# suryatmodulus/livekit-server

Measured on AMD Instinct MI355X. Metric: forwarded RTP pkts/sec per GPU & node (bit-exact) + % HBM roofline, higher is better.
Workload: dtype u8; 1 GPU; configs[1]: 100 rooms x 10 participants per GPU, VP8 3-layer simulcast + Opus, 18000 DownTracks, 2% loss, 1% reorder, layer switching; batch=1 s of media per step, step=raw datagrams -> Buffer.calc -> forward (lkf_ingest_device + lkf_run), parallelism=room-sharded x1

## Files before the change

livekit-server_amd/csrc/engine.cpp:

```cpp
#include <hip/hip_runtime.h>

#include <algorithm>
#include <chrono>
#include <cmath>
#include <cstdio>
#include <cstdlib>
#include <cstring>
#include <atomic>
#include <map>
#include <memory>
#include <mutex>
#include <string>
#include <tuple>
#include <vector>

#include "../../include/lkfwd.h"
#include "ctl_csr.h"
#include "dev_buf.h"
#include "fwd_state.h"
#include "handles.h"
#include "hip_own.h"
#include "kernels.h"

using namespace lkf;
// ... 5128 lines not shown
    HIPCHK(hipStreamSynchronize(e->ingS), "sync ingest stream");
    HIPCHK(hipStreamSynchronize(e->decS), "sync decide stream");
    release_all(e->dRsRowEng, e->dRsSlotOff, e->dRsSlotDts, e->dRsSlotSub);
    HIPCHK(e->dRsRowEng.alloc(rowEng.size()), "alloc");
    HIPCHK(e->dRsSlotOff.alloc(off.size()), "alloc");
    HIPCHK(e->dRsSlotDts.alloc(dts.size()), "alloc");
    HIPCHK(e->dRsSlotSub.alloc(sub.size()), "alloc");
    HIPCHK(hipMemcpy(e->dRsRowEng, rowEng.data(), rowEng.size() * 4, hipMemcpyHostToDevice), "copy");
    HIPCHK(hipMemcpy(e->dRsSlotOff, off.data(), off.size() * 4, hipMemcpyHostToDevice), "copy");
    HIPCHK(hipMemcpy(e->dRsSlotDts, dts.data(), dts.size() * 4, hipMemcpyHostToDevice), "copy");
    HIPCHK(hipMemcpy(e->dRsSlotSub, sub.data(), sub.size() * 8, hipMemcpyHostToDevice), "copy");
    e->rsRooms = rooms;
    e->rsK = k;
    e->rsS = s;
    e->rsGen = e->topoGen;
  }
  hipStream_t cs = reinterpret_cast<hipStream_t>(stream);
  if (e->nRooms) {
    SpeakersLaunch a;
    a.nrooms = e->nRooms;
    a.roomPartOff = e->dRoomPartOff;
    a.partId = e->dPartId;
    a.partMicOff = e->dPartMicOff;
    a.mics = e->dMics;
    a.roomId = e->dRoomId;
    a.streams = e->dStreams;
    a.hot = e->dStreamHot;
    a.nowNs = now_ns;
    a.slots = e->dSpkSlots;
    a.counts = e->dSpkCounts;
    HIPCHK(launch_speakers(e->ingS, a), "speakers");
  }
  RoomPackLaunch p;
  p.rows = rows;
  p.k = k;
  p.s = s;
  p.rowEng = e->dRsRowEng;
  p.slots = e->dSpkSlots;
  p.counts = e->dSpkCounts;
  p.slotOff = e->dRsSlotOff;
  p.slotDts = e->dRsSlotDts;
  p.slotSub = e->dRsSlotSub;
  p.cum = e->dDTCum;
  p.spk = spk;
  p.bwe = bwe;
  HIPCHK(launch_room_pack(e->ingS, e->decS, p), "room pack");
  HIPCHK(hipEventRecord(e->rsSpk, e->ingS), "event");
  HIPCHK(hipEventRecord(e->rsDec, e->decS), "event");
  HIPCHK(hipStreamWaitEvent(cs, e->rsSpk, 0), "wait");
  HIPCHK(hipStreamWaitEvent(cs, e->rsDec, 0), "wait");
  return LKF_OK;
}

int lkf_debug_svc_stats(lkf_engine *e, uint64_t out[48], int reset) {
  if (!e || !out) return LKF_EINVAL;
  int rc = drain_streams(e);
  if (rc) return rc;
  unsigned long long v[48];
  const hipError_t r = read_svc_stats(v, reset);
  for (int i = 0; i < 48; i++) out[i] = v[i];
  return r == hipSuccess ? LKF_OK : LKF_ENODEV;
}

int lkf_debug_check(lkf_engine *e, uint64_t out[4], int reset) {
  if (!out) return LKF_EINVAL;
  if (e) {
    int rc = drain_streams(e);
    if (rc) return rc;
  } else if (hipDeviceSynchronize() != hipSuccess) {
    return LKF_EHIP;
  }
  unsigned long long v[4];
  hipError_t r = read_check(v, reset);
  for (int i = 0; i < 4; i++) out[i] = v[i];
  {
    unsigned long long w[4];
    if (read_check_rtcp(w, reset) == hipSuccess && w[0]) {
      if (!out[0]) out[1] = w[1], out[2] = w[2], out[3] = w[3];
      out[0] += w[0];
    }
  }
  std::atomic<uint64_t> &ctr = e ? e->rangeViolations : gRangeViolationsAll;
  const uint64_t rv = reset ? ctr.exchange(0) : ctr.load();
  if (rv) {
    if (!out[0]) out[1] = 0xD2, out[2] = 0, out[3] = 0;
    out[0] += rv;
    return LKF_OK;
  }
  return r == hipSuccess ? LKF_OK : LKF_ENODEV;
}

int lkf_debug_dd_cursors(lkf_engine *e, uint64_t out[7]) {
  if (!e || !out || !e->ddAlloc) return LKF_EINVAL;
  STEP(quiesce(e, false));
  for (int c = 0; c < lkf_engine::kCtx; c++) {
    uint64_t u[2] = {0, 0};
    D2H(u, e->ctx[c].dDDUsed, sizeof(u), "dd cursor copy");
    out[2 * c] = u[0];
    out[2 * c + 1] = u[1] & 0xffffffffu;
  }
  out[6] = e->ctx[0].dDDArena.cap();
  return LKF_OK;
}

int lkf_debug_dd_state(lkf_engine *e, int32_t dt, uint64_t out[16]) {
  if (!e || !out || dt < 0 || size_t(dt) >= e->dtp.size() || !e->dDDState) return LKF_EINVAL;
  STEP(quiesce(e, false));
  DDState d;
  DTHot h;
  D2H(&d, e->dDDState + dt, sizeof(d), "dd state");
  D2H(&h, e->dHot + dt, sizeof(h), "hot state");
  out[0] = (d.flags & DS_CACHE_INIT) ? 1 : 0;
  out[1] = d.cBase;
// ... 59 lines not shown
```

livekit-server_amd/csrc/forward_kernels.hip:

```cpp
#include <hip/hip_runtime.h>

#include "../../include/lkfwd.h"
#ifndef LKF_SVC_STATS
#define LKF_SVC_STATS 0
#endif
#if LKF_SVC_STATS
__device__ unsigned long long g_svc[64 * 48];
#define SVC_ADD(k, v) atomicAdd(&g_svc[(blockIdx.x & 63) * 48 + (k)], (unsigned long long)(v))
#endif
#include "dd_device.h"
#include "fwd_state.h"
#include "kernels.h"
#include "sender_device.h"

namespace lkf {

using u8 = uint8_t;
using u16 = uint16_t;
using u32 = uint32_t;
using u64 = uint64_t;
using i32 = int32_t;
using i64 = int64_t;

constexpr u64 HALF64 = 1ull << 63;
constexpr i32 INVALID = -1;


#ifndef LKF_CHECKED
#define LKF_CHECKED 0
#endif
#if LKF_CHECKED
__device__ unsigned long long g_chk[4];
__device__ __noinline__ void chk_fail(u32 site, u64 idx, u64 cap) {
  if (atomicAdd(&g_chk[0], 1ull) == 0) {
    g_chk[1] = site;
    g_chk[2] = idx;
    g_chk[3] = cap;
  }
}
#define CHK(cond, site, idx, cap)                   \
  do {                                              \
    if (!(cond)) chk_fail(site, u64(idx), u64(cap)); \
  } while (0)
#else
#define CHK(cond, site, idx, cap) \
  do {                            \
  } while (0)
#endif
enum ChkSite : u32 {
  CK_DEC_DT = 1,
  CK_DEC_TRACK,
  CK_DEC_PKT,
  CK_DEC_TUPLE,
  CK_DEC_SEQ,
  CK_DEC_LAYER,
  CK_DEC_EVENT,
  CK_EMIT_POS,
  CK_EMIT_DT,
  CK_EMIT_TUPLE,
  CK_EMIT_PKT,
  CK_EMIT_ARENA,
// ... 671 lines not shown
      L.h.ptgtT = L.h.tgtT = i32(ev.a[1]);
      break;
    case LKF_CTL_PLAYOUT_ACKED:
      setf(L, F_PLAYOUT_ACKED, ev.a[0] != 0);
      break;
    case kOpLayerOffsets: {
      const u32 l = lane_id();
      if (l < 9) L.offs[l] = l < 8 ? u32(u64(ev.a[l >> 1]) >> (32 * (l & 1))) : u32(u64(ev.pad));
      break;
    }
    default:
      break;
  }
}

__device__ bool fw_sourceSwitch(Lane &L, const PktV &p, i32 layer) {
  if (!hasf(L, F_STARTED)) {
    setf(L, F_STARTED, true);
    L.h.referenceLayerSpatial = layer;
    mg_setLastSnTs(L, p.esn, p.ets);
    if (hasf(L, F_VP8)) vp8_setLast(L, p);
    return true;
  } else if (L.h.referenceLayerSpatial == INVALID) {
    L.h.referenceLayerSpatial = layer;
  }
  const u64 extLastTS = L.h.extLastTS;
  u64 extExpectedTS = extLastTS;
  u64 extRefTS = extExpectedTS;
  if (L.hasRefTS) {
    i32 ref = L.h.referenceLayerSpatial;
    if (layer < 0 || layer >= 3 || ref < 0 || ref >= 3) return false;
    const bool svc = L.codec == LKF_CODEC_VP9 || L.codec == LKF_CODEC_AV1;
    const u32 off = svc ? 0u : L.offs[ref * 3 + layer];
    if (!svc && layer != ref && off == 0) return false;
    u32 ts = u32(p.ets) + off;
    extRefTS = (extRefTS & 0xFFFFFFFF00000000ull) + u64(ts);
    u32 e32 = u32(extExpectedTS);
    if (u32(ts - e32) < (1u << 31) && ts < e32) extRefTS += (1ull << 32);
    if (u32(e32 - ts) < (1u << 31) && e32 < ts && extRefTS >= (1ull << 32)) extRefTS -= (1ull << 32);
  }
  if (hasf(L, F_HAS_EXPECTED)) {
    if (hasf(L, F_STATS_INIT)) {
      i64 diff = (p.arr - L.h.statsFirstTime) * i64(L.clockRate) / 1000000000LL;
      extExpectedTS = L.h.statsExtStartTS + u64(diff);
    } else if (L.h.preStartTime != 0) {
      i64 since = p.arr - L.h.preStartTime;
      u64 rtpDiff = u64(since * i64(L.clockRate) / 1000000000LL);
      extExpectedTS = L.h.extFirstTS + rtpDiff;
      if (L.h.refTSOffset == 0) L.h.refTSOffset = extExpectedTS - extRefTS;
    }
  }
  extRefTS += L.h.refTSOffset;
  u64 extNextTS;
  const double cr = double(L.clockRate);
  if (L.h.lastSSRC == 0) {
    double diffSeconds = double(i64(extExpectedTS - extRefTS)) / cr;
    if (diffSeconds >= 0.0) {
      if (hasf(L, F_RESUME_BEHIND) && diffSeconds > 0.2)
        extNextTS = extExpectedTS;
      else if (diffSeconds > 2.0)
        extNextTS = extExpectedTS;
      else
        extNextTS = extRefTS;
    } else {
      extNextTS = extRefTS;
    }
    setf(L, F_RESUME_BEHIND, false);
  } else {
    double diffSeconds = double(i64(extRefTS - extLastTS)) / cr;
    if (diffSeconds < 0.0) {
      if (fabs(diffSeconds) > 0.05) return false;
      extNextTS = extLastTS + 1;
    } else {
      extNextTS = extRefTS;
    }
  }
  if (i64(extNextTS - extLastTS) <= 0) extNextTS = extLastTS + 1;
  mg_updateSnTsOffsets(L, p.esn, p.ets, 1, extNextTS - extLastTS);
  if (hasf(L, F_VP8)) vp8_updateOffsets(L, p);
  return true;
}

__device__ __forceinline__ int fw_common(Lane &L, const PktV &p, i32 layer, bool marker, int &ord, u64 &osn,
                                         u64 &ots) {
  if (L.h.lastSSRC != p.ssrc) {
    if (!fw_sourceSwitch(L, p, layer)) return LKF_DROP_SWITCH;
    L.h.lastSSRC = p.ssrc;
  }
  int r = mg_update(L, p, marker, ord, osn, ots);
  if (r == MG_PADDING) return LKF_DROP_PADDING;
  if (r == MG_DUP) return LKF_DROP_DUPLICATE;
  if (r == MG_OOO_MISS) return LKF_DROP_OOO_MISS;
  return -1;
}

template <bool DDK = false>
__device__ __forceinline__ void vls_rollback(Lane &L) {
  if (DDK && hasf(L, F_DD)) {
    L.dd->mask = L.dd->prevMask;
    if (L.dd->flags & DS_HAS_PREV_MASK)
      L.dd->flags |= DS_HAS_MASK;
    else
      L.dd->flags &= ~u32(DS_HAS_MASK);
  }
  L.h.curS = L.h.prevS;
  L.h.curT = L.h.prevT;
  L.h.tgtS = L.h.ptgtS;
// ... 1015 lines not shown
__device__ __forceinline__ void pin_loaded(const uint4 &a, const uint4 &b, const uint4 &c, const uint4 &d) {
  asm volatile("" ::"v"(a.x), "v"(a.y), "v"(a.z), "v"(a.w), "v"(b.x), "v"(b.y), "v"(b.z), "v"(b.w), "v"(c.x),
               "v"(c.y), "v"(c.z), "v"(c.w), "v"(d.x), "v"(d.y), "v"(d.z), "v"(d.w));
}

__device__ __forceinline__ void relaunder(uint4 &a, uint4 &b, uint4 &c, uint4 &d) {
  asm volatile("" : "+v"(a.x), "+v"(a.y), "+v"(a.z), "+v"(a.w), "+v"(b.x), "+v"(b.y), "+v"(b.z), "+v"(b.w),
                 "+v"(c.x), "+v"(c.y), "+v"(c.z), "+v"(c.w), "+v"(d.x), "+v"(d.y), "+v"(d.z), "+v"(d.w));
}

__device__ __forceinline__ bool steady_state(const Lane &L) {
  const u32 fl = L.h.flags;
  return (fl & F_VIDEO) && (fl & F_SIMULCAST) && !(fl & (F_MUTED | F_PUBMUTED)) &&
         L.h.tgtS != INVALID && L.h.tgtT != INVALID && L.h.curS == L.h.tgtS && L.h.curS <= L.h.maxS &&
         L.h.curS >= 0 && L.h.curS < 3;
}

__global__ void __launch_bounds__(64) k_layer_index(const RunDesc *__restrict__ desc, const u32 *__restrict__ tBegin,
                                                    const u32 *__restrict__ tEnd, u32 stride, u32 *__restrict__ list,
                                                    u32 *__restrict__ before, u32 *__restrict__ cnt,
                                                    u64 *__restrict__ zero2) {
  const lkf_pkt *__restrict__ pkts = reinterpret_cast<const lkf_pkt *>(desc->pkts);
  const u32 t = blockIdx.x, lane = threadIdx.x;
  if (zero2 && t == 0 && lane < 2) zero2[lane] = 0;
  const u64 lt = (1ull << lane) - 1;
  const u32 b = tBegin[t], e = tEnd[t];
  u32 c0 = 0, c1 = 0, c2 = 0;
  for (u32 base = b; base < e; base += 64) {
    const u32 i = base + lane;
    const int l = i < e ? int(reinterpret_cast<const int8_t *>(pkts + i)[53]) : -1;
    const u64 m0 = __ballot(l == 0), m1 = __ballot(l == 1), m2 = __ballot(l == 2);
    if (i < e) {
      const u32 r0 = c0 + u32(__popcll(m0 & lt)), r1 = c1 + u32(__popcll(m1 & lt)), r2 = c2 + u32(__popcll(m2 & lt));
      before[i] = r0;
      before[stride + i] = r1;
      before[2 * size_t(stride) + i] = r2;
      if (l == 0) list[b + r0] = i;
      if (l == 1) list[stride + b + r1] = i;
      if (l == 2) list[2 * size_t(stride) + b + r2] = i;
    }
    c0 += u32(__popcll(m0));
    c1 += u32(__popcll(m1));
    c2 += u32(__popcll(m2));
  }
  if (lane == 0) {
    cnt[t * 3] = c0;
    cnt[t * 3 + 1] = c1;
    cnt[t * 3 + 2] = c2;
  }
}

#ifndef LKF_SVC_CHAINS
#define LKF_SVC_CHAINS 1
#endif
constexpr int kSvcDDBytes = 48;
constexpr int kSvcFrames = 72;
enum : u32 { SK_BAD = 0, SK_FWD = 1, SK_MDROP = 2, SK_NDROP = 3 };

#if LKF_SVC_STATS
#define SVC_WHY(c) \
  if (why == 0 && inWin && !good) why = (c)
#else
#define SVC_WHY(c)
#endif

template <bool DDK>
__device__ __forceinline__ u32 svc_run(Lane &L, LaneOut &o, const PktV &p, u32 pi, u32 n, u32 pos, u32 nextAt,
                                       bool valid, i32 &sentAcc, u8 *sScr, u8 *sFD) {
  const u32 lane = lane_id();
  const u64 lt = (1ull << lane) - 1;
  const u32 fl = L.h.flags;
  const bool inWin = valid && lane >= pos && pi < nextAt;
  const u64 winM = __ballot(inWin);
  const bool dd = DDK && (fl & F_DD);
  {
    const int ns = (fl & (F_MUTED | F_PUBMUTED)) ? LKF_DROP_MUTED
                   : (L.h.tgtS == INVALID || L.h.tgtT == INVALID) ? LKF_DROP_PAUSED
                                                                  : -1;
    if (ns >= 0) {
      const u32 k = u32(__popcll(winM));
      o.nTuples += k;
      if (ns == LKF_DROP_MUTED)
        o.drops[LKF_DROP_MUTED] += k;
      else
        o.drops[LKF_DROP_PAUSED] += k;
      return pos + k;
    }
  }
  const bool curValid = L.h.curS != INVALID && L.h.curT != INVALID;
  const bool started = fl & F_STARTED;
  const bool relevantDrop = curValid && started;
  bool uni = true;
  const DDStruct *s = nullptr;
  int hiPos = -1, maxTgt = -1;
  u32 hiTarget = 0;
  bool swAll = false;
  u32 aboveM = 0, hiChain = 0xffffffffu;
  if (DDK && dd) {
    const DDState &d = *L.dd;
    uni = (d.flags & DS_KF_VALID) && (d.flags & DS_CACHE_INIT);
    uni = uni && u32(d.slot) == L.ddSSlot;
    s = L.ddS;
    for (int i = 0; uni && i < int(d.numTargets); i++) {
      if (!((d.dtActive >> i) & 1) || i32(s->dtS[i]) > L.h.tgtS || i32(s->dtT[i]) > L.h.tgtT) continue;
      const int target = s->dtTarget[i];
      maxTgt = max(maxTgt, target);
// ... 717 lines not shown
    const bool steady = pe - pb > 64 && steady_state(L);
    u32 pi, n, lim;
    if (steady) {
      const u32 ls = u32(L.h.curS);
      CHK(size_t(ls) * A->pktStride + kpos < 3 * size_t(A->pktStride), CK_DEC_LAYER, size_t(ls) * A->pktStride + kpos,
          3 * size_t(A->pktStride));
      const u32 j = A->layerBefore[size_t(ls) * A->pktStride + kpos] + lane;
      pi = j < A->layerCnt[track * 3 + ls] ? A->layerList[size_t(ls) * A->pktStride + pb + j] : 0xffffffffu;
      const u32 stopAt = min(nextAt, pe);
      n = u32(__popcll(__ballot(pi < stopAt)));
      lim = n == 64 ? rl32(pi, 63) + 1 : stopAt;
    } else {
      n = min(64u, pe - kpos);
      pi = kpos + lane;
      lim = kpos + n;
    }
    const bool valid = lane < n;
    if (!pre) {
      r0 = r1 = r2 = r3 = make_uint4(0, 0, 0, 0);
      if (valid) {
        CHK(pi < A->npkts, CK_DEC_PKT, pi, A->npkts);
        const u64 q = u64(pi) * 4;
        r0 = src[q];
        r1 = src[q + 1];
        r2 = src[q + 2];
        r3 = src[q + 3];
      }
    }
    pre = false;
    pin_loaded(r0, r1, r2, r3);
#if LKF_SVC_STATS
    {
      u64 tl0;
      const u32 dep = __builtin_amdgcn_readfirstlane(r0.x ^ r3.w);
      asm volatile("s_memtime %0\n s_waitcnt lgkmcnt(0)" : "=s"(tl0) : "s"(dep));
      tLoad += tl0 - tc0;
    }
#endif
    u32 pos = 0;
    u32 own = n;
    while (pos < n) {
      relaunder(r0, r1, r2, r3);
      const PktV p = decode_pkt(r0, r1, r2, r3);
      if (nextAt <= rl32(pi, pos)) {
        const DecideArgsK A = decide_args();
        while (nextAt <= rl32(pi, pos)) {
          apply_ctl(L, A->events[ev++]);
          nextAt = ev < evEnd ? A->events[ev].at : 0xffffffffu;
        }
        vm_drain();
      }
      u32 x;
      bool gapStop = false;
      if (DDK && svcDT) {
#if LKF_SVC_STATS
        const u64 tr0 = __builtin_amdgcn_s_memtime();
#endif
        x = svc_run<DDK>(L, o, p, pi, n, pos, nextAt, valid, sentAcc, sSvcScr, sSvcFD);
        pos = x;
#if LKF_SVC_STATS
        const u64 tr1 = __builtin_amdgcn_s_memtime();
        tRun += tr1 - tr0;
#endif
        if (x < n && rl32(pi, x) < nextAt) {
          const u32 px = rl32(pi, x);
          decide_step<DDK>(L, load_pkt(pkts + px), px, o);
          vm_drain();
          if (ddDT) dd_restage(L, sDD, sDDSRaw, lane);
#if LKF_SVC_STATS
          tStep += __builtin_amdgcn_s_memtime() - tr1;
#endif
#if LKF_SVC_STATS
          if (lane == 0) SVC_ADD(2, 1ull);
#endif
          pos = x + 1;
        }
        continue;
      } else {
      const bool inWin = valid && lane >= pos && pi < nextAt;
      const u32 fl = L.h.flags;
      const bool video = fl & F_VIDEO;
      const i32 layer = p.layer;
      const bool kf = p.flags & LKF_PKT_KEYFRAME;
      const bool pktMarker = p.hdr1 & 0x80;
      int cls;
      if (fl & (F_MUTED | F_PUBMUTED)) {
        cls = LKF_DROP_MUTED;
      } else if (!video) {
        cls = -1;
      } else if (L.h.tgtS == INVALID || L.h.tgtT == INVALID) {
        cls = LKF_DROP_PAUSED;
      } else if (!(fl & F_SIMULCAST)) {
        cls = (fl & (F_VP9 | F_DD)) ? -2 : LKF_DROP_NOT_SELECTED;
      } else {
        const bool willSwitch =
            kf && ((L.h.curS != L.h.tgtS && ((layer > L.h.curS && layer <= L.h.tgtS) ||
                                             (layer < L.h.curS && layer >= L.h.tgtS))) ||
                   (L.h.curS > L.h.maxS && layer <= L.h.maxS));
        if (willSwitch)
          cls = -2;
        else if (layer != L.h.curS)
          cls = LKF_DROP_NOT_SELECTED;
        else if ((fl & F_DEFICIENT) && L.h.tgtS < L.h.curS)
          cls = LKF_DROP_DOWNGRADE;
        else if ((fl & F_VP8) && (fl & F_TLS_VP8) && (p.flags & LKF_PKT_VP8))
          cls = -1;
        else
          cls = -2;
      }
      const bool cand = inWin && cls == -1;
      const bool candIn = cand;
      const u64 candM = __ballot(candIn);
      const int pc = prev_in(candM, lt);
      const int pcs = pc >= 0 ? pc : int(lane);
      const u64 pcEsn = sh64(p.esn, pcs);
      const u64 prevEsn = pc >= 0 ? pcEsn : L.h.extHighestIncomingSN;
      const u64 dEsn = p.esn - prevEsn;
      const bool gapLane = candIn && dEsn > 1 && dEsn < u64(L.seqSize) - 64 &&
                           p.plen != 0 && p.ssrc == L.h.lastSSRC;
      bool ok = candIn && (dEsn == 1 || gapLane) && p.plen != 0 && p.ssrc == L.h.lastSSRC;
      const bool gapLater = candIn && pc >= 0 && dEsn > 1 && dEsn < u64(L.seqSize) - 64 && p.plen != 0 &&
                            p.ssrc == L.h.lastSSRC;
      const bool M = p.vbits & LKF_VP8_M, I = p.vbits & LKF_VP8_I, T = p.vbits & LKF_VP8_T;
      const i32 np = M ? i32(p.pid & 0x7fff) : i32(p.pid & 0x7f);
      const i32 ext = np + L.h.wrTotalWrap;
      const i32 pcExt = i32(sh32(u32(ext), pcs));
      const bool pcM = sh32(u32(M), pcs) != 0;
      const i32 prevExt = pc >= 0 ? pcExt : L.h.wrMaxPictureId;
      const bool prevM = pc >= 0 ? pcM : ((fl & F_WR_MAX_MBIT) != 0);
      bool dropT = false;
      u64 tswM = 0;
      bool overT = false;
      if (video) {
        i32 mp = prevExt;
        if (mp > 0) mp = prevM ? (prevExt & 0x7fff) : (prevExt & 0x7f);
        const bool wrapBack = L.h.wrTotalWrap > 0 && (prevExt + (L.h.wrLastWrap >> 1)) < (np + L.h.wrTotalWrap);
        const bool wraps = np < mp && (mp - np) > (prevM ? (1 << 14) : (1 << 6));
        const i32 cT = L.h.curT, gT = L.h.tgtT;
        const bool tsw = cT != gT && T &&
                         (cT < gT ? (i32(p.tid) > cT && i32(p.tid) <= gT && (p.vbits & LKF_VP8_S) &&
                                     (p.vbits & LKF_VP8_Y))
                                  : pktMarker);
        overT = candIn && T && p.tid > u8(cT);
        bool exIn = false;
        for (u64 ge = __ballot(gapLane && overT); ge; ge &= ge - 1) {
          const u32 k = u32(__ffsll((long long)ge) - 1);
          exIn = exIn || (lane > k && ext == i32(rl32(u32(ext), k)));
        }
        dropT = overT && !gapLane && !exIn;
        if (__ballot(dropT) && L.h.exCount)
          dropT = dropT && !set_has(L.exKey, L.h.exHead, L.h.exCount, ext);
        if (tsw && cT < gT) dropT = false;
        const bool tswOk = tsw && !gapLane && !dropT;
        ok = ok && !wrapBack && !wraps && (!tsw || tswOk) && (!dropT || L.h.snOffset == L.h.rmOpenValue);
        tswM = __ballot(inWin && ok && tsw);
      }
      const u64 tdM = __ballot(ok && dropT);
      const u64 snOff = L.h.snOffset + u64(__popcll(tdM & lt));
      u64 osn = p.esn - snOff;
      const u64 ots = p.ets - L.h.tsOffset;
      const bool picDrop = ok && dropT && I && ext != prevExt;
      const i32 picOff = L.h.pictureIdOffset + i32(__popcll(__ballot(picDrop) & lt));
      const bool fwdIn = ok && !dropT;
      const i32 mext = ext - picOff;
      const u16 mpid = u16(mext & 0x7fff);
      const u8 mtl0 = u8(p.tl0 - L.h.tl0Off);
      const u8 mkey = u8((p.keyidx - L.h.keyIdxOff) & 0x1f);
      u64 cb = 0;
      int cbLen = 0;
      if (video) {
        const bool mM = mpid > 127;
        const int hs = int(p.vhs) + (mM == M ? 0 : (mM ? 1 : -1));
        cbLen = vp8_marshal(p.vfirst, I, mM, mpid, p.vbits & LKF_VP8_L, mtl0, T, p.tid, p.vbits & LKF_VP8_Y,
                            p.vbits & LKF_VP8_K, mkey, hs, cb);
      }
      const u64 fwC = __ballot(fwdIn);
      const int pf = prev_in(fwC, lt);
      const int pfs = pf >= 0 ? pf : int(lane);
      const u64 pfOsn = sh64(osn, pfs);
      const u64 prevOsn = pf >= 0 ? pfOsn : L.h.seqExtHighestSN;
      const u64 pfOts = sh64(ots, pfs);
      const u64 hiTS = pf >= 0 ? pfOts : L.h.seqExtHighestTS;
      bool fwd = fwdIn;
      const bool tsMono = ots >= hiTS;
      const bool seqOk = (fl & F_SEQ_INIT) && (fl & F_STATS_INIT) && cbLen >= 0 && tsMono &&
                         (osn == prevOsn + 1 || (gapLane && osn - prevOsn > 1 &&
                                                 osn - prevOsn < u64(L.seqSize) - 64)) &&
                         osn - L.h.seqExtHighestSN < u64(L.seqSize) - 64;
      const bool bad =
          inWin && ((cls == -2) || (cls == -1 && !ok) || (fwdIn && !seqOk));
      const u64 stopM = __ballot(bad || (valid && lane >= pos && !inWin));
      x = stopM ? u32(__ffsll((long long)stopM) - 1) : n;
      if (tswM & ~((1ull << pos) - 1)) x = min(x, u32(__ffsll((long long)(tswM & ~((1ull << pos) - 1))) - 1) + 1u);
      if (x > pos) {
        const u64 runM = (x >= 64 ? ~0ull : ((1ull << x) - 1)) & ~((1ull << pos) - 1);
        const bool inRun = (runM >> lane) & 1;
        const u64 tdR = tdM & runM;
        fwd = fwd && inRun;
        const u64 fwR = __ballot(fwd);
        const u64 fwInR = fwR;
        const u64 selR = tdR | fwInR;
        o.nTuples += x - pos;
        o.drops[LKF_DROP_MUTED] += u32(__popcll(__ballot(inRun && cls == LKF_DROP_MUTED)));
        o.drops[LKF_DROP_PAUSED] += u32(__popcll(__ballot(inRun && cls == LKF_DROP_PAUSED)));
        o.drops[LKF_DROP_NOT_SELECTED] += u32(__popcll(__ballot(inRun && cls == LKF_DROP_NOT_SELECTED)));
        o.drops[LKF_DROP_DOWNGRADE] += u32(__popcll(__ballot(inRun && cls == LKF_DROP_DOWNGRADE)));
        o.drops[LKF_DROP_TEMPORAL] += u32(__popcll(tdR));
        const u64 pdR = video ? __ballot(picDrop && inRun) : 0ull;
        const u64 gR = __ballot(gapLane && inRun);
        if (gR) {
          for (u64 m = gR | pdR; m; m &= m - 1) {
            const u32 b = u32(__ffsll((long long)m) - 1);
            const i32 eb = i32(rl32(u32(ext), b));
            if ((pdR >> b) & 1) {
              L.vcDirty = true;
              set_add(L.dropKey, L.h.dropHead, L.h.dropCount, eb, kDropKeep);
              continue;
            }
            if (video) {
              vp8_record_missing(L, i32(rl32(u32(prevExt), b)), eb, i32(rl32(u32(picOff), b)));
              if (rl32(u32(overT), b)) {
                L.vcDirty = true;
                set_add(L.exKey, L.h.exHead, L.h.exCount, eb, kExemptKeep);
              }
            }
            const u64 from = rl64(prevOsn, b), to = rl64(osn, b);
            const u32 n = u32(to - from - 1);
            u32 base = u32(L.h.seqHighSlot) + u32(from - L.h.seqExtHighestSN) + 1;
            for (u32 i = lane; i < n; i += 64) {
              u32 x2 = base + i;
              while (x2 >= L.seqSize) x2 -= L.seqSize;
              store_rec(L.seq + x2, SeqMeta{});
            }
          }
        }
        const int cc = p.hdr0 & 0xf;
        const bool playout = L.extPlayout && !(fl & F_PLAYOUT_ACKED);
        const int extBytes = (playout ? 4 : 0) + (L.extAbs ? 4 : 0) + (L.extTcc ? 3 : 0);
        const int extBlock = extBytes ? 4 + ((extBytes + 3) & ~3) : 0;
        const int hdrLen = 12 + 4 * cc + extBlock;
        const bool useCodec = video && cbLen > 0 && (p.flags & LKF_PKT_VP8);
        const int payLen = useCodec ? (cbLen + int(p.plen) - int(p.vhs)) : int(p.plen);
        const u32 outLen = fwd ? u32(hdrLen + payLen) : 0u;
        const u32 aligned = (outLen + 15) & ~15u;
        const u32 relEx = excl_scan_u32(aligned, lane);
        const bool marker = pktMarker;
        const u32 j = u32(__popcll(fwR & lt));
        fwd_base(o, fwR, osn, ots);
        if (fwd) {
#if LKF_CHECKED
          CHK(slot0 + o.nFwd + j < A->tupleCap, CK_DEC_TUPLE, slot0 + o.nFwd + j, A->tupleCap);
#endif
          store_fwd(o.outT + o.nFwd + j, o.outW + o.nFwd + j, o.bSN, o.bTS, osn, ots, pi, o.relOff + relEx, outLen,
                    ((p.flags & LKF_PKT_KEYFRAME) ? LKF_OUT_KEYFRAME : 0) | (marker ? LKF_OUT_MARKER : 0) |
                        (playout ? T_PLAYOUT : 0) | (useCodec ? T_CODEC : 0),
                    0u, useCodec ? vp8_aux(mpid, mtl0, mkey) : 0u);
          u32 slot = u32(L.h.seqHighSlot) + u32(osn - L.h.seqExtHighestSN);
          while (slot >= L.seqSize) slot -= L.seqSize;
          SeqMeta m = {};
          m.sourceSeqNo = u16(p.esn);
          m.targetSeqNo = u16(osn);
          m.timestamp = u32(ots);
          m.lastNack = u32(p.arr / 1000000LL - L.h.seqStartMs);
          m.marker = marker;
          m.layer = p.layer;
          m.codecLen = u8(video ? cbLen : 0);
#pragma unroll
          for (int i = 0; i < 8; i++) m.codec[i] = u8(cb >> (8 * i));
          CHK(slot < L.seqSize, CK_DEC_SEQ, slot, L.seqSize);
          store_rec(L.seq + slot, m);
        }
        if (fwd) ss_put(o.ssBuf + o.ssN + j, o, u32(o.nFwd) + j, osn, ots, p.arr, p.poff, u32(payLen), marker, kf);
        o.ssN += u32(__popcll(fwR));
        const u32 sumLen = wave_sum_u32(outLen);
        sentAcc += fwd ? i32(p.poff) - hdrLen : 0;
        if (fwR) {
          o.nBytes += sumLen;
          o.nFwd += u32(__popcll(fwR));
        }
        if (fwInR) {
          const u32 lastF = 63 - __clzll(fwInR);
          u32 slot = u32(L.h.seqHighSlot) + u32(rl64(osn, lastF) - L.h.seqExtHighestSN);
          while (slot >= L.seqSize) slot -= L.seqSize;
          L.h.seqHighSlot = u16(slot);
          L.h.seqExtHighestSN = rl64(osn, lastF);
          L.h.seqExtHighestTS = rl64(ots, lastF);
          if (video) {
            L.h.extLastPictureId = i32(rl32(u32(mext), lastF));
            L.h.lastTl0 = u8(rl32(mtl0, lastF));
            L.h.lastKeyIdx = u8(rl32(mkey, lastF));
          }
        }
        if (selR) {
          const u32 lastSel = 63 - __clzll(selR);
          const u64 mk = __ballot(video && pktMarker);
          L.h.extHighestIncomingSN = rl64(p.esn, lastSel);
          const bool lastIsF = (fwInR >> lastSel) & 1;
          const u64 pfM = fwInR & ((1ull << lastSel) - 1);
          u64 sSN = L.h.extLastSN, sTS = L.h.extLastTS;
          bool sMk = fl & F_LAST_MARKER;
          if (pfM) {
            const u32 b = 63 - __clzll(pfM);
            sSN = rl64(osn, b);
            sTS = rl64(ots, b);
            sMk = (mk >> b) & 1;
          }
          if (lastIsF) {
            L.h.extSecondLastSN = sSN;
            L.h.extSecondLastTS = sTS;
            L.h.extLastSN = rl64(osn, lastSel);
            L.h.extLastTS = rl64(ots, lastSel);
            setf(L, F_SECOND_LAST_MARKER, sMk);
            setf(L, F_LAST_MARKER, (mk >> lastSel) & 1);
          } else {
            L.h.extSecondLastSN = L.h.extLastSN = sSN;
            L.h.extSecondLastTS = L.h.extLastTS = sTS;
            setf(L, F_SECOND_LAST_MARKER, sMk);
            setf(L, F_LAST_MARKER, sMk);
          }
          if (hasf(L, F_RTX_GATE) && (rl64(osn, lastSel) - L.h.extRtxGateSn) > 2000) setf(L, F_RTX_GATE, false);
          const u64 kfM = __ballot(((selR >> lane) & 1) && kf);
          if (kfM) {
            L.h.extRtxGateSn = rl64(osn, 63 - __clzll(kfM));
            setf(L, F_RTX_GATE, true);
          }
          if (video) {
            L.h.wrMaxPictureId = i32(rl32(u32(ext), lastSel));
            setf(L, F_WR_MAX_MBIT, rl32(u32(M), lastSel) != 0);
            u64 m = tdR;
            while (m) {
              const u32 b = u32(__ffsll((long long)m) - 1);
              const u64 after = fwInR & ~((2ull << b) - 1);
              const u32 nf = after ? u32(__ffsll((long long)after) - 1) : 64u;
              const u64 runD = tdR & (nf >= 64 ? ~0ull : ((1ull << nf) - 1)) & ~((1ull << b) - 1);
              const u64 s0 = rl64(p.esn, b);
              rm_exclude(L, s0, s0 + u64(__popcll(runD)));
              m &= ~runD;
            }
            if (tdR) L.h.snOffset = L.h.rmOpenValue;
            const u64 tswR = tswM & runM;
            if (tswR) {
              const u32 b = 63 - __clzll(tswR);
              const i32 nxt = L.h.curT < L.h.tgtT ? i32(rl32(u32(p.tid), b)) : L.h.tgtT;
              L.h.prevS = L.h.curS;
              L.h.prevT = L.h.curT;
              L.h.curT = nxt;
            }
            u64 pd = pdR;
            L.h.pictureIdOffset += i32(__popcll(pd));
            while (pd && !gR) {
              const u32 b = u32(__ffsll((long long)pd) - 1);
              L.vcDirty = true;
              set_add(L.dropKey, L.h.dropHead, L.h.dropCount, i32(rl32(u32(ext), b)), kDropKeep);
              pd &= pd - 1;
            }
          }
        }
        if (fwR) o.relOff += rl32(relEx + aligned, 63 - __clzll(fwR));
      }
      gapStop = x < n && rl32(u32(gapLater), x) != 0;
      }
      pos = x;
      if (x < n && rl32(pi, x) < nextAt && !gapStop) {
        const uint4 a0 = make_uint4(rl32(r0.x, x), rl32(r0.y, x), rl32(r0.z, x), rl32(r0.w, x));
        const uint4 a1 = make_uint4(rl32(r1.x, x), rl32(r1.y, x), rl32(r1.z, x), rl32(r1.w, x));
        const uint4 a2 = make_uint4(rl32(r2.x, x), rl32(r2.y, x), rl32(r2.z, x), rl32(r2.w, x));
        const uint4 a3 = make_uint4(rl32(r3.x, x), rl32(r3.y, x), rl32(r3.z, x), rl32(r3.w, x));
        const u32 px = rl32(pi, x);
        decide_step<DDK>(L, decode_pkt(a0, a1, a2, a3), px, o);
        vm_drain();
        if (DDK && ddDT) dd_restage(L, sDD, sDDSRaw, lane);
        pos = x + 1;
        if (steady && !steady_state(L)) {
          own = x + 1;
          lim = px + 1;
          break;
        }
      }
    }
    if (steady) {
      const u32 skipped = (lim - kpos) - own;
      o.nTuples += skipped;
      o.drops[LKF_DROP_NOT_SELECTED] += skipped;
    }
    if (o.ssN) {
      wave_lds_sync();
#if LKF_SVC_STATS
      const u64 ts0 = __builtin_amdgcn_s_memtime();
#endif
      ss_flush(sSS, o.ssRing, o.ssGap, sSsBuf, o.ssN, o.bSN, o.bTS, o.outW);
#if LKF_SVC_STATS
      tSs += __builtin_amdgcn_s_memtime() - ts0;
#endif
      o.ssN = 0;
    }
    kpos = lim;
  }
#if LKF_SVC_STATS
  const u64 tP2 = __builtin_amdgcn_s_memtime();
#endif
  {
  const DecideArgsK A = decide_args();
  while (ev < evEnd) apply_ctl(L, A->events[ev++]);
  __syncthreads();
  {
    const u32 h1 = reinterpret_cast<const u32 *>(&sHot)[lane];
    if (h1 != sHot0[lane]) reinterpret_cast<u32 *>(A->hot + d)[lane] = h1;
  }
  if (o.nFwd && lane < sizeof(SenderStats) / 16)
    reinterpret_cast<uint4 *>(A->ss + d)[lane] = reinterpret_cast<const uint4 *>(&sSS)[lane];
  if (L.rmNew) {
    wave_lds_sync();
    const u32 nc = L.h.rmCount, nn = min(L.rmNew, nc);
    for (u32 i = lane; i < nn; i += 64) {
      const u32 idx = (u32(L.h.rmHead) + nc - nn + i) % kRangeCap;
      rmG[idx] = sRm[idx];
// ... 1221 lines not shown
      }
      if (a < 64) {
        if (__builtin_amdgcn_readlane(int(attOK), a)) {
          st.cur = next;
          st.valid = 1;
          updates++;
        }
        pend &= ~((2ull << a) - 1);
      } else {
        pend = 0;
      }
    }
    if (isDD) out[i] = o;
    if (trk != 0xffffffffu) {
      const u64 vM = __ballot(isDD && (o.flags & DP_VALID));
      const u32 w0 = u32(o.flags) | (u32(o.slot) << 8) | (u32(o.ndti) << 16) | (u32(r.flags) << 24);
      for (u64 w = vM; w; w &= w - 1) {
        const u32 x = u32(__ffsll(static_cast<long long>(w)) - 1);
        const u32 fx = u32(__builtin_amdgcn_readlane(int(w0), x));
        const u32 amx = u32(__builtin_amdgcn_readlane(int(o.activeMask), x));
        const u64 dtx = (u64(u32(__builtin_amdgcn_readlane(int(u32(o.dtis >> 32)), x))) << 32) |
                        u32(__builtin_amdgcn_readlane(int(u32(o.dtis)), x));
        const u32 szx = u32(__builtin_amdgcn_readlane(int(psize), x));
        const u32 pyx = u32(__builtin_amdgcn_readlane(int(pay), x));
        if (lane == 0) {
          DDPkt q = {};
          q.flags = u8(fx);
          q.slot = u8(fx >> 8);
          q.ndti = u8(fx >> 16);
          q.activeMask = amx;
          q.dtis = dtx;
          dd_tracker_observe(ddTrk[trk], ring[q.slot], q, fx >> 24, szx, pyx);
        }
      }
    }
  }
  if (updates > u32(kDDSlots / 2)) bad = true;
  if (__ballot(bad) && lane == 0) atomicOr(err, 16u);
  if (lane == 0) ddTracks[ddIdx] = st;
}

hipError_t launch_dd_decode(hipStream_t s, const RunDesc *desc, const uint32_t *tBegin, const uint32_t *tEnd,
                            const DevTrack *tracks, uint32_t ntracks, DDStruct *structs, DDTrack *ddTracks, DDPkt *out,
                            uint32_t *err, const uint32_t *trackDDTrk, DDTrkState *ddTrk, uint16_t *spill,
                            uint32_t *spillUsed, uint32_t spillCap) {
  if (!ntracks) return hipSuccess;
  hipLaunchKernelGGL(k_dd_decode, dim3(ntracks), dim3(64), 0, s, desc, tBegin, tEnd, tracks, ntracks, structs,
                     ddTracks, out, err, trackDDTrk, ddTrk, spill, spillUsed, spillCap);
  return hipGetLastError();
}

static u32 nblk(u64 n, u32 t) { return u32((n + t - 1) / t); }

hipError_t read_svc_stats(unsigned long long out[48], int reset) {
#if LKF_SVC_STATS
  static unsigned long long v[64 * 48];
  hipError_t r = hipMemcpyFromSymbol(v, HIP_SYMBOL(g_svc), sizeof(v));
  for (int k = 0; k < 48; k++) {
    out[k] = 0;
    for (int c = 0; c < 64; c++) out[k] += v[c * 48 + k];
  }
  if (r == hipSuccess && reset) {
    for (auto &x : v) x = 0;
    r = hipMemcpyToSymbol(HIP_SYMBOL(g_svc), v, sizeof(v));
  }
  return r;
#else
  for (int i = 0; i < 48; i++) out[i] = 0;
  (void)reset;
  return hipErrorNotSupported;
#endif
}

hipError_t read_check(unsigned long long out[4], int reset) {
#if LKF_CHECKED
  hipError_t r = hipMemcpyFromSymbol(out, HIP_SYMBOL(g_chk), sizeof(unsigned long long) * 4);
  if (r == hipSuccess && reset) {
    unsigned long long z[4] = {};
    r = hipMemcpyToSymbol(HIP_SYMBOL(g_chk), z, sizeof(z));
  }
  return r;
#else
  (void)reset;
  for (int i = 0; i < 4; i++) out[i] = 0;
  return hipErrorNotSupported;
#endif
}

hipError_t launch_batch_init(hipStream_t s, u32 ntracks, u32 ndts, u32 nstats, u32 *tBegin, u32 *tEnd, u32 *tRuns,
                             u32 *err, u64 *stats, u32 *fwdCnt, u64 *fwdBytes) {
  u32 n = ntracks > ndts ? ntracks : ndts;
  if (n < nstats) n = nstats;
  u32 g = nblk(n, 256);
  if (g > 1024) g = 1024;
  hipLaunchKernelGGL(k_batch_init, dim3(g), dim3(256), 0, s, ntracks, ndts, nstats, tBegin, tEnd, tRuns, err, stats,
                     fwdCnt, fwdBytes);
  return hipGetLastError();
}

hipError_t launch_track_ranges(hipStream_t s, const RunDesc *desc, u32 maxPkts, u32 ntracks, u32 *tBegin, u32 *tEnd,
                               u32 *tRuns, u32 *err) {
  if (maxPkts == 0) return hipSuccess;
  hipLaunchKernelGGL(k_track_ranges, dim3(nblk(maxPkts, 256)), dim3(256), 0, s, desc, ntracks, tBegin, tEnd, tRuns,
                     err);
  return hipGetLastError();
}

hipError_t launch_scan(hipStream_t s, int mode, const DevDT *dts, const u32 *tBegin, const u32 *tEnd, const u32 *cnt,
                       const u64 *bytes, u32 n, u64 *partA, u64 *partB, u64 *outA, u64 *outB, u64 *totA, u64 *totB,
                       const u32 *perm, u32 *gFirst, u64 gCap) {
  (void)partB;
  ScanIn in;
  in.gFirst = gFirst;
  in.gCap = gCap;
  in.mode = mode;
  in.perm = perm;
  in.dts = dts;
  in.tBegin = tBegin;
  in.tEnd = tEnd;
  in.cnt = cnt;
  in.bytes = bytes;
// ... 192 lines not shown
```

livekit-server_amd/csrc/kernels.h:

```cpp
#pragma once
#include <hip/hip_runtime.h>

#include "../../include/lkfwd.h"
#include "fps_dd_device.h"
#include "fps_device.h"
#include "fwd_state.h"
#include "srtcp_device.h"
#include "srtp_rx_device.h"

namespace lkf {

struct DecideArgs {
  const uint32_t *sched;
  const uint32_t *waveTrack;
  uint32_t nlanes;
  DTHot *hot;
  const DevDT *dts;
  const DevTrack *tracks;
  RangeEntry *rm;
  VP8Cold *vc;
  SeqMeta *seq;
  uint32_t seqSize;
  uint8_t *srm;
  uint64_t srmStride;
// ... 10 lines not shown
  uint32_t *ssRing, *ssGap;
  uint32_t *dtOffs;
  const DevEvent *events;
  const uint32_t *evOff;
  uint32_t *fwdCnt;
  uint64_t *fwdBytes;
  DTCum *dtCum;
  uint64_t *stats;
  const uint32_t *layerList, *layerBefore, *layerCnt;
  uint32_t pktStride;
  uint32_t waveBase;
  uint32_t waveEnd;
  uint32_t perWave;
  const DDPkt *ddPkts;
  const DDStruct *ddStructs;
  DDState *ddState;
  uint8_t *ddArena;
  uint64_t *ddUsed;
  uint64_t ddCap;
  const uint16_t *ddSpill;
  uint32_t maxDts, maxTracks, npkts, nev;
};

struct EmitArgs {
  const uint32_t *perm;
  const uint64_t *recBase;
  const uint64_t *byteBase;
  const uint32_t *gFirst;
  const uint64_t *slotBase;
  const uint64_t *totals;
  const FwdRec *recs;
  const FwdBase *fbase;
  const FwdBase *wide;
  const lkf_pkt *pkts;
  const uint8_t *arena;
  const DevDT *dts;
  uint32_t ndts;
  lkf_out *out;
  uint8_t *outArena;
  uint64_t outCap, outByteCap;
  uint32_t *err;
  const uint8_t *ddArena;
  const uint32_t *twccBase;
  uint32_t maxDts, npkts;
  uint64_t tupleCap, arenaLen, ddCap, gCap;
};
hipError_t launch_twcc_base(hipStream_t s, const DevDT *dts, uint32_t ndts, const uint32_t *fwdCnt, uint32_t *ctrD,
                            uint32_t *ctrT, const uint32_t *tOff, const uint32_t *tList, uint32_t ntr,
                            uint32_t *base);
hipError_t launch_twcc_stamp(hipStream_t s, const DevDT *dts, uint32_t *ctrD, uint32_t *ctrT, uint32_t n,
                             const lkf_out *recs, const uint64_t *recOff, const uint32_t *cnt, const lkf_rtx *rtx,
                             const uint64_t *off, const uint32_t *len, uint8_t *arena);
hipError_t read_check(unsigned long long out[4], int reset);
hipError_t read_svc_stats(unsigned long long out[48], int reset);

hipError_t launch_batch_init(hipStream_t s, uint32_t ntracks, uint32_t ndts, uint32_t nstats, uint32_t *tBegin,
                             uint32_t *tEnd, uint32_t *tRuns, uint32_t *err, uint64_t *stats, uint32_t *fwdCnt,
                             uint64_t *fwdBytes);
hipError_t launch_track_ranges(hipStream_t s, const RunDesc *desc, uint32_t maxPkts, uint32_t ntracks,
                               uint32_t *tBegin, uint32_t *tEnd, uint32_t *tRuns, uint32_t *err);
size_t scan_state_words(uint32_t maxN);
hipError_t launch_scan(hipStream_t s, int mode, const DevDT *dts, const uint32_t *tBegin, const uint32_t *tEnd,
                       const uint32_t *cnt, const uint64_t *bytes, uint32_t n, uint64_t *partA, uint64_t *partB,
                       uint64_t *outA, uint64_t *outB, uint64_t *totA, uint64_t *totB,
                       const uint32_t *perm, uint32_t *gFirst = nullptr, uint64_t gCap = 0);
struct BucketLaunch;
struct NackIn {
  int64_t arrival;
  uint32_t stream;
  uint32_t snFl;
  uint32_t s0, len;
};
static_assert(sizeof(NackIn) == 24, "24 B per datagram");
constexpr uint32_t kNackFastPairs = 256;
struct IngestLaunch {
  const lkf_raw_pkt *raws;
  uint32_t n;
  const uint8_t *raw;
  const DevStream *streams;
  uint32_t nstreams, ntracks;
  StreamHot *hot;
  uint64_t *hist;
  uint32_t *rxGap;
  RangeEntry *rings;
  IngParsed *parsed;
  uint32_t *tBegin, *tEnd, *tRuns, *err;
  lkf_flow *flows;
  uint32_t *fwd;
  uint32_t *twcc;
  uint64_t *pos, *partA, *partB, *total;
  lkf_pkt *out;
  DDIngState *ddStates;
  DDStruct *ddStructs;
  IngDD *ingDD;
  lkf_pkt_dd *outDD;
  uint32_t *list, *listCnt;
  uint32_t listStride;
  NackState *nack;
  uint32_t *nackInfo, *nackPairOff, *nackPairCnt;
  lkf_nack_pair *nackPairs;
  uint32_t nackPairCap;
  NackIn *nackIn;
  uint32_t nfps = 0;
  const uint32_t *fpsList = nullptr;
  uint32_t *fpsCalcAt = nullptr;
  fps::State *fpsStates = nullptr;
  uint32_t fpsEpoch = 0;
// ... 482 lines not shown
```

Before: 1.566 billion forwarded RTP pkts/s.

## Handle out-of-order late packets inside wave-parallel forwarding runs

Packets that arrive late (reordered, sequence number below the previous candidate) used to end a wave-wide run and drop back to the serial per-packet decide step. Up to four ballot passes now mark late lanes and exclude them from the prev-candidate chain. Each late lane is then resolved in-run: the range-map offset, OOO/picture-ID miss drops and the VP8 header re-marshal are computed, so the run can continue. It also pins the clock rate to a scalar register with an empty asm and widens the debug stats counters. The cost is more ballots and a serial loop over late lanes, plus a risk to bit-exact output in the new paths.

```diff
diff --git a/livekit-server_amd/csrc/engine.cpp b/livekit-server_amd/csrc/engine.cpp
--- a/livekit-server_amd/csrc/engine.cpp
+++ b/livekit-server_amd/csrc/engine.cpp
@@ -5204,13 +5204,13 @@
   return LKF_OK;
 }
 
-int lkf_debug_svc_stats(lkf_engine *e, uint64_t out[48], int reset) {
+int lkf_debug_svc_stats(lkf_engine *e, uint64_t out[64], int reset) {
   if (!e || !out) return LKF_EINVAL;
   int rc = drain_streams(e);
   if (rc) return rc;
-  unsigned long long v[48];
+  unsigned long long v[64];
   const hipError_t r = read_svc_stats(v, reset);
-  for (int i = 0; i < 48; i++) out[i] = v[i];
+  for (int i = 0; i < 64; i++) out[i] = v[i];
   return r == hipSuccess ? LKF_OK : LKF_ENODEV;
 }
 
diff --git a/livekit-server_amd/csrc/forward_kernels.hip b/livekit-server_amd/csrc/forward_kernels.hip
--- a/livekit-server_amd/csrc/forward_kernels.hip
+++ b/livekit-server_amd/csrc/forward_kernels.hip
@@ -5,8 +5,8 @@
 #define LKF_SVC_STATS 0
 #endif
 #if LKF_SVC_STATS
-__device__ unsigned long long g_svc[64 * 48];
-#define SVC_ADD(k, v) atomicAdd(&g_svc[(blockIdx.x & 63) * 48 + (k)], (unsigned long long)(v))
+__device__ unsigned long long g_svc[64 * 64];
+#define SVC_ADD(k, v) atomicAdd(&g_svc[(blockIdx.x & 63) * 64 + (k)], (unsigned long long)(v))
 #endif
 #include "dd_device.h"
 #include "fwd_state.h"
@@ -784,7 +784,9 @@
   }
   extRefTS += L.h.refTSOffset;
   u64 extNextTS;
-  const double cr = double(L.clockRate);
+  u32 crU = L.clockRate;
+  asm volatile("" : "+s"(crU));
+  const double cr = double(crU);
   if (L.h.lastSSRC == 0) {
     double diffSeconds = double(i64(extExpectedTS - extRefTS)) / cr;
     if (diffSeconds >= 0.0) {
@@ -1906,6 +1908,9 @@
 
 #ifndef LKF_SVC_CHAINS
 #define LKF_SVC_CHAINS 1
+#endif
+#ifndef LKF_OOO_RUN
+#define LKF_OOO_RUN 1
 #endif
 constexpr int kSvcDDBytes = 48;
 constexpr int kSvcFrames = 72;
@@ -2729,6 +2734,9 @@
       }
       u32 x;
       bool gapStop = false;
+#if LKF_SVC_STATS
+      u32 whyStop = 0;
+#endif
       if (DDK && svcDT) {
 #if LKF_SVC_STATS
         const u64 tr0 = __builtin_amdgcn_s_memtime();
@@ -2786,12 +2794,23 @@
           cls = -2;
       }
       const bool cand = inWin && cls == -1;
-      const bool candIn = cand;
-      const u64 candM = __ballot(candIn);
-      const int pc = prev_in(candM, lt);
-      const int pcs = pc >= 0 ? pc : int(lane);
-      const u64 pcEsn = sh64(p.esn, pcs);
-      const u64 prevEsn = pc >= 0 ? pcEsn : L.h.extHighestIncomingSN;
+      u64 candM = __ballot(cand);
+      int pc = prev_in(candM, lt);
+      int pcs = pc >= 0 ? pc : int(lane);
+      u64 pcEsn = sh64(p.esn, pcs);
+      u64 prevEsn = pc >= 0 ? pcEsn : L.h.extHighestIncomingSN;
+      bool late = false;
+#if LKF_OOO_RUN
+      for (int pass = 0; pass < 4 && __ballot(cand && !late && i64(p.esn - prevEsn) < 0); pass++) {
+        late = late || (cand && i64(p.esn - prevEsn) < 0);
+        candM = __ballot(cand && !late);
+        pc = prev_in(candM, lt);
+        pcs = pc >= 0 ? pc : int(lane);
+        pcEsn = sh64(p.esn, pcs);
+        prevEsn = pc >= 0 ? pcEsn : L.h.extHighestIncomingSN;
+      }
+#endif
+      const bool candIn = cand && !late;
       const u64 dEsn = p.esn - prevEsn;
       const bool gapLane = candIn && dEsn > 1 && dEsn < u64(L.seqSize) - 64 &&
                            p.plen != 0 && p.ssrc == L.h.lastSSRC;
@@ -2808,6 +2827,7 @@
       bool dropT = false;
       u64 tswM = 0;
       bool overT = false;
+      bool lateBad = false;
       if (video) {
         i32 mp = prevExt;
         if (mp > 0) mp = prevM ? (prevExt & 0x7fff) : (prevExt & 0x7f);
@@ -2831,6 +2851,7 @@
         const bool tswOk = tsw && !gapLane && !dropT;
         ok = ok && !wrapBack && !wraps && (!tsw || tswOk) && (!dropT || L.h.snOffset == L.h.rmOpenValue);
         tswM = __ballot(inWin && ok && tsw);
+        lateBad = wrapBack || wraps || tsw;
       }
       const u64 tdM = __ballot(ok && dropT);
       const u64 snOff = L.h.snOffset + u64(__popcll(tdM & lt));
@@ -2840,7 +2861,7 @@
       const i32 picOff = L.h.pictureIdOffset + i32(__popcll(__ballot(picDrop) & lt));
       const bool fwdIn = ok && !dropT;
       const i32 mext = ext - picOff;
-      const u16 mpid = u16(mext & 0x7fff);
+      u16 mpid = u16(mext & 0x7fff);
       const u8 mtl0 = u8(p.tl0 - L.h.tl0Off);
       const u8 mkey = u8((p.keyidx - L.h.keyIdxOff) & 0x1f);
       u64 cb = 0;
@@ -2864,29 +2885,22 @@
                          (osn == prevOsn + 1 || (gapLane && osn - prevOsn > 1 &&
                                                  osn - prevOsn < u64(L.seqSize) - 64)) &&
                          osn - L.h.seqExtHighestSN < u64(L.seqSize) - 64;
+      const bool lateOk = LKF_OOO_RUN && late && !lateBad && p.plen != 0 && p.ssrc == L.h.lastSSRC &&
+                          (fl & F_SEQ_INIT) && (fl & F_STATS_INIT) && !(fl & F_SEQ_RM) && ots <= hiTS;
       const bool bad =
-          inWin && ((cls == -2) || (cls == -1 && !ok) || (fwdIn && !seqOk));
+          inWin && ((cls == -2) || (cls == -1 && !ok && !lateOk) || (fwdIn && !seqOk));
       const u64 stopM = __ballot(bad || (valid && lane >= pos && !inWin));
       x = stopM ? u32(__ffsll((long long)stopM) - 1) : n;
       if (tswM & ~((1ull << pos) - 1)) x = min(x, u32(__ffsll((long long)(tswM & ~((1ull << pos) - 1))) - 1) + 1u);
       if (x > pos) {
-        const u64 runM = (x >= 64 ? ~0ull : ((1ull << x) - 1)) & ~((1ull << pos) - 1);
-        const bool inRun = (runM >> lane) & 1;
-        const u64 tdR = tdM & runM;
-        fwd = fwd && inRun;
-        const u64 fwR = __ballot(fwd);
-        const u64 fwInR = fwR;
-        const u64 selR = tdR | fwInR;
-        o.nTuples += x - pos;
-        o.drops[LKF_DROP_MUTED] += u32(__popcll(__ballot(inRun && cls == LKF_DROP_MUTED)));
-        o.drops[LKF_DROP_PAUSED] += u32(__popcll(__ballot(inRun && cls == LKF_DROP_PAUSED)));
-        o.drops[LKF_DROP_NOT_SELECTED] += u32(__popcll(__ballot(inRun && cls == LKF_DROP_NOT_SELECTED)));
-        o.drops[LKF_DROP_DOWNGRADE] += u32(__popcll(__ballot(inRun && cls == LKF_DROP_DOWNGRADE)));
-        o.drops[LKF_DROP_TEMPORAL] += u32(__popcll(tdR));
-        const u64 pdR = video ? __ballot(picDrop && inRun) : 0ull;
-        const u64 gR = __ballot(gapLane && inRun);
-        if (gR) {
-          for (u64 m = gR | pdR; m; m &= m - 1) {
+        u64 runM = (x >= 64 ? ~0ull : ((1ull << x) - 1)) & ~((1ull << pos) - 1);
+        bool inRun = (runM >> lane) & 1;
+        u64 pdR = video ? __ballot(picDrop && inRun) : 0ull;
+        u64 gR = __ballot(gapLane && inRun);
+        u64 lateR = LKF_OOO_RUN ? __ballot(late && inRun) : 0ull;
+        const bool ordered = (gR | lateR) != 0;
+        if (ordered) {
+          for (u64 m = gR | pdR | lateR; m; m &= m - 1) {
             const u32 b = u32(__ffsll((long long)m) - 1);
             const i32 eb = i32(rl32(u32(ext), b));
             if ((pdR >> b) & 1) {
@@ -2894,6 +2908,72 @@
               set_add(L.dropKey, L.h.dropHead, L.h.dropCount, eb, kDropKeep);
               continue;
             }
+#if LKF_OOO_RUN
+            if ((lateR >> b) & 1) {
+              const u64 key = rl64(p.esn, b);
+              const u64 below = (1ull << b) - 1;
+              const u64 tdB = tdM & runM & below;
+              const u64 sameM = __ballot(p.esn == key) & (fwC | tdM | lateR) & runM & below;
+              const u64 pfM = fwC & runM & below;
+              int dr = -1;
+              u64 lsn = 0, lcb = 0;
+              int lcbLen = 0;
+              u16 lpid = 0;
+              if (sameM & ~tdB) {
+                dr = -2;
+              } else if (sameM) {
+                dr = LKF_DROP_OOO_MISS;
+              } else {
+                if (key < L.h.rmOpenStart) dr = -2;
+                if (dr == -1) {
+                  lsn = key - (L.h.rmOpenValue + u64(__popcll(__ballot(((tdB >> lane) & 1) && p.esn < key))));
+                  const u64 lastF = pfM ? rl64(osn, 63 - __clzll(pfM)) : 0ull;
+                  const u64 lastSN = pfM ? lastF : L.h.extLastSN, seqHi = pfM ? lastF : L.h.seqExtHighestSN;
+                  const u64 fwRun = fwC & runM;
+                  const u64 reach = fwRun ? rl64(osn, 63 - __clzll(fwRun)) : L.h.seqExtHighestSN;
+                  if (lsn >= lastSN)
+                    dr = LKF_DROP_OOO_MISS;
+                  else if (lsn < L.h.seqExtStartSN || i64(lsn - seqHi) >= 0 || i64(lsn - reach) <= -i64(L.seqSize))
+                    dr = -2;
+                }
+                if (dr == -1 && video) {
+                  const int idx = miss_find(L, eb);
+                  if (idx < 0) {
+                    dr = LKF_DROP_PICID_MISS;
+                  } else {
+                    const u32 vb = rl32(u32(p.vbits), b);
+                    lpid = u16((eb - L.missVal[idx]) & 0x7fff);
+                    const bool lM = lpid > 127, oM = vb & LKF_VP8_M;
+                    const int hs = int(rl32(u32(p.vhs), b)) + (lM == oM ? 0 : (lM ? 1 : -1));
+                    lcbLen = vp8_marshal(u8(rl32(u32(p.vfirst), b)), vb & LKF_VP8_I, lM, lpid, vb & LKF_VP8_L,
+                                         u8(rl32(u32(p.tl0), b) - L.h.tl0Off), vb & LKF_VP8_T, u8(rl32(u32(p.tid), b)),
+                                         vb & LKF_VP8_Y, vb & LKF_VP8_K, u8(rl32(u32(p.keyidx), b) - L.h.keyIdxOff),
+                                         hs, lcb);
+                    if (lcbLen < 0) dr = LKF_DROP_OTHER;
+                  }
+                }
+              }
+#if LKF_SVC_STATS
+              if (lane == 0) SVC_ADD(dr == -2 ? 54 : dr == -1 ? 52 : 53, 1ull);
+#endif
+              if (dr == -2) {
+                x = b;
+                runM &= below;
+                break;
+              }
+              o.drops[LKF_DROP_OOO_MISS] += dr == LKF_DROP_OOO_MISS ? 1u : 0u;
+              o.drops[LKF_DROP_PICID_MISS] += dr == LKF_DROP_PICID_MISS ? 1u : 0u;
+              o.drops[LKF_DROP_OTHER] += dr == LKF_DROP_OTHER ? 1u : 0u;
+              if (dr == -1 && lane == b) {
+                fwd = true;
+                osn = lsn;
+                cb = lcb;
+                cbLen = lcbLen;
+                mpid = lpid;
+              }
+              continue;
+            }
+#endif
             if (video) {
               vp8_record_missing(L, i32(rl32(u32(prevExt), b)), eb, i32(rl32(u32(picOff), b)));
               if (rl32(u32(overT), b)) {
@@ -2910,7 +2990,25 @@
               store_rec(L.seq + x2, SeqMeta{});
             }
           }
+          if (lateR) {
+            inRun = (runM >> lane) & 1;
+            pdR &= runM;
+            gR &= runM;
+            lateR &= runM;
+            vm_drain();
+          }
         }
+        const u64 tdR = tdM & runM;
+        fwd = fwd && inRun;
+        const u64 fwR = __ballot(fwd);
+        const u64 fwInR = fwR & ~lateR;
+        const u64 selR = tdR | fwInR;
+        o.nTuples += x - pos;
+        o.drops[LKF_DROP_MUTED] += u32(__popcll(__ballot(inRun && cls == LKF_DROP_MUTED)));
+        o.drops[LKF_DROP_PAUSED] += u32(__popcll(__ballot(inRun && cls == LKF_DROP_PAUSED)));
+        o.drops[LKF_DROP_NOT_SELECTED] += u32(__popcll(__ballot(inRun && cls == LKF_DROP_NOT_SELECTED)));
+        o.drops[LKF_DROP_DOWNGRADE] += u32(__popcll(__ballot(inRun && cls == LKF_DROP_DOWNGRADE)));
+        o.drops[LKF_DROP_TEMPORAL] += u32(__popcll(tdR));
         const int cc = p.hdr0 & 0xf;
         const bool playout = L.extPlayout && !(fl & F_PLAYOUT_ACKED);
         const int extBytes = (playout ? 4 : 0) + (L.extAbs ? 4 : 0) + (L.extTcc ? 3 : 0);
@@ -2933,6 +3031,7 @@
                         (playout ? T_PLAYOUT : 0) | (useCodec ? T_CODEC : 0),
                     0u, useCodec ? vp8_aux(mpid, mtl0, mkey) : 0u);
           u32 slot = u32(L.h.seqHighSlot) + u32(osn - L.h.seqExtHighestSN);
+          if (LKF_OOO_RUN && i32(slot) < 0) slot += L.seqSize;
           while (slot >= L.seqSize) slot -= L.seqSize;
           SeqMeta m = {};
           m.sourceSeqNo = u16(p.esn);
@@ -3025,7 +3124,7 @@
             }
             u64 pd = pdR;
             L.h.pictureIdOffset += i32(__popcll(pd));
-            while (pd && !gR) {
+            while (pd && !ordered) {
               const u32 b = u32(__ffsll((long long)pd) - 1);
               L.vcDirty = true;
               set_add(L.dropKey, L.h.dropHead, L.h.dropCount, i32(rl32(u32(ext), b)), kDropKeep);
@@ -3036,9 +3135,21 @@
         if (fwR) o.relOff += rl32(relEx + aligned, 63 - __clzll(fwR));
       }
       gapStop = x < n && rl32(u32(gapLater), x) != 0;
+#if LKF_SVC_STATS
+      if (lane == 0) SVC_ADD(48, 1ull);
+      if (x < n)
+        whyStop = rl32((cand && (late || i64(p.esn - prevEsn) < 0) ? 1u : 0u) | (cand && p.esn == prevEsn ? 2u : 0u), x);
+#endif
       }
       pos = x;
       if (x < n && rl32(pi, x) < nextAt && !gapStop) {
+#if LKF_SVC_STATS
+        if (!DDK && lane == 0) {
+          SVC_ADD(49, 1ull);
+          if (whyStop & 1) SVC_ADD(50, 1ull);
+          if (whyStop & 2) SVC_ADD(51, 1ull);
+        }
+#endif
         const uint4 a0 = make_uint4(rl32(r0.x, x), rl32(r0.y, x), rl32(r0.z, x), rl32(r0.w, x));
         const uint4 a1 = make_uint4(rl32(r1.x, x), rl32(r1.y, x), rl32(r1.z, x), rl32(r1.w, x));
         const uint4 a2 = make_uint4(rl32(r2.x, x), rl32(r2.y, x), rl32(r2.z, x), rl32(r2.w, x));
@@ -4366,13 +4477,13 @@
 
 static u32 nblk(u64 n, u32 t) { return u32((n + t - 1) / t); }
 
-hipError_t read_svc_stats(unsigned long long out[48], int reset) {
+hipError_t read_svc_stats(unsigned long long out[64], int reset) {
 #if LKF_SVC_STATS
-  static unsigned long long v[64 * 48];
+  static unsigned long long v[64 * 64];
   hipError_t r = hipMemcpyFromSymbol(v, HIP_SYMBOL(g_svc), sizeof(v));
-  for (int k = 0; k < 48; k++) {
+  for (int k = 0; k < 64; k++) {
     out[k] = 0;
-    for (int c = 0; c < 64; c++) out[k] += v[c * 48 + k];
+    for (int c = 0; c < 64; c++) out[k] += v[c * 64 + k];
   }
   if (r == hipSuccess && reset) {
     for (auto &x : v) x = 0;
@@ -4380,7 +4491,7 @@
   }
   return r;
 #else
-  for (int i = 0; i < 48; i++) out[i] = 0;
+  for (int i = 0; i < 64; i++) out[i] = 0;
   (void)reset;
   return hipErrorNotSupported;
 #endif
diff --git a/livekit-server_amd/csrc/kernels.h b/livekit-server_amd/csrc/kernels.h
--- a/livekit-server_amd/csrc/kernels.h
+++ b/livekit-server_amd/csrc/kernels.h
@@ -86,7 +86,7 @@
                              const lkf_out *recs, const uint64_t *recOff, const uint32_t *cnt, const lkf_rtx *rtx,
                              const uint64_t *off, const uint32_t *len, uint8_t *arena);
 hipError_t read_check(unsigned long long out[4], int reset);
-hipError_t read_svc_stats(unsigned long long out[48], int reset);
+hipError_t read_svc_stats(unsigned long long out[64], int reset);
 
 hipError_t launch_batch_init(hipStream_t s, uint32_t ntracks, uint32_t ndts, uint32_t nstats, uint32_t *tBegin,
                              uint32_t *tEnd, uint32_t *tRuns, uint32_t *err, uint64_t *stats, uint32_t *fwdCnt,
```

Result: faster. 1.611 billion forwarded RTP pkts/s (median of 6 runs) (+2.9%).
